# FSSRepo/ggml-cuda-experiments

Hardware: AMD Instinct MI355X
Metric: attn TFLOPS & HBM GB/s per GPU; head_dim=128 seq=4096 Q8_0 KV (higher is better)
Workload: dtype f16; 1 GPU; decode_q8_0_h32_hkv32_d128_n4096_q1; heads=32, kv_heads=32, head_dim=128, kv_len=4096, n_q=1, kv_type=q8_0, kv_layout=head, kv_rotation=16, parallelism=single_gpu

## Files before the change

ggml-cuda-experiments_amd/csrc/fattn_api.hip:

```cpp
#include <hip/hip_runtime.h>

#include <algorithm>
#include <atomic>
#include <cmath>
#include <cstdio>
#include <cstdlib>
#include <cstring>
#include <type_traits>

#include "fattn_plan.h"

using namespace fattn;

namespace {

constexpr int kCUsDefault = 256;

int device_cus() {
    static std::atomic<int> cache[kMaxDevices];
    int dev = 0;
    if (hipGetDevice(&dev) != hipSuccess || dev < 0 || dev >= kMaxDevices) {
        (void)hipGetLastError();
        return kCUsDefault;
    }
// ... 136 lines not shown
            std::snprintf(kern, sizeof kern, "%s<%s,D%d,%s>%s%s", pl.kernel == Kernel::Bdp ? "fattn_bdp_kernel" : "fattn_bd_kernel",
                          tn(pl.kt), pl.D, hm, xcd, merge);
            break;
        case Kernel::Mq:
            if (pl.a.merge_launch)
                std::snprintf(merge, sizeof merge, " + fattn_mq_merge_kernel%s", pl.a.part_f16 ? "(f16 partials)" : "");
            std::snprintf(kern, sizeof kern, "fattn_mq_kernel<%s,D%d,%dwaves,%s>%s", tn(pl.kt), pl.D, pl.nw, hm, merge);
            break;
        case Kernel::Split:
        case Kernel::SplitLd: {
            const bool ld = pl.kernel == Kernel::SplitLd;
            merged_by("fattn_merge_kernel");
            std::snprintf(kern, sizeof kern, "%s<%s,%s,D%d,gran%d,%s,%dwaves%s>%s%s", ld ? "fattn_split_ld_kernel" : "fattn_split_kernel",
                          tn(pl.kt), tn(pl.vt), pl.D, pl.gran, hm, pl.nwv, ld ? "+4loaders" : "", xcd, merge);
            break;
        }
    }
    char planes[48] = "";
    if (pl.a.m_ne2 > 1 || pl.a.m_ne3 > 1) std::snprintf(planes, sizeof planes, " mask planes (%d,%d)", pl.a.m_ne2, pl.a.m_ne3);
    char xf[64] = "";
    int xn = 0;
    if (pl.a.xf.live & 1) xn = std::snprintf(xf, sizeof xf, " softcap %g", (double)p->logit_softcap);
    if (pl.a.xf.live & 2) std::snprintf(xf + xn, sizeof xf - xn, " alibi %g", (double)p->max_bias);
    const int n = std::snprintf(out, cap, "%s grid(%u,%u,%u) lds %d chunk %d steps/slots %d ws %zu%s%s", kern, pl.grid.x,
                                pl.grid.y, pl.grid.z, pl.lds, pl.a.chunk_len, pl.a.nbuf, pl.ws_bytes, planes, xf);
    return n < 0 || (size_t)n >= cap ? FATTN_ERR_INVALID_ARG : FATTN_OK;
}

}

namespace {

int launch_ext(const fattn_params* p, const float* sinks, void* stream, void* ev_begin, void* ev_end) {
    Plan pl;
    const int rc = plan_now(p, pl);
    if (rc != FATTN_OK) return rc;
    if ((uintptr_t)sinks % 4) return FATTN_ERR_ALIGNMENT;
    pl.a.sinks = sinks;
    if (pl.ws_bytes) {
        if (!p->workspace || p->workspace_bytes < pl.ws_bytes || (uintptr_t)p->workspace % 16) return FATTN_ERR_WORKSPACE;
        uint8_t* w = (uint8_t*)p->workspace;
        pl.a.ws_cnt = (uint32_t*)w;
        uint32_t e = g_epoch.fetch_add(1, std::memory_order_relaxed) + 1;
        if (e == 0) e = g_epoch.fetch_add(1, std::memory_order_relaxed) + 1;
        pl.a.arrival_stamp = kArrivalTag | (uint64_t)e << kArrivalEpochShift;
        pl.a.ws_ml = (float*)(w + pl.cnt_bytes);
        pl.a.ws_o = (float*)(w + pl.cnt_bytes + pl.ml_bytes);
        if (pl.pf_flags) pl.a.pf_flags = w;
        if (pl.pf_stage) {
            pl.a.k = w + pl.stage_off;
            pl.a.v = w + pl.stage_off + pl.stage_bytes;
        }
    }
    hipStream_t st = (hipStream_t)stream;
    Events ev;
    ev.begin = (hipEvent_t)ev_begin;
    ev.end = (hipEvent_t)ev_end;
    if (pl.kernel == Kernel::Mla) return launch_mla(pl, st, ev);
    switch (pl.D) {
        case 64: return launch_types<64>(pl, st, ev);
        case 80: return launch_types<80>(pl, st, ev);
        case 96: return launch_types<96>(pl, st, ev);
        case 128: return launch_types<128>(pl, st, ev);
        default: return launch_types<256>(pl, st, ev);
    }
}

}

extern "C" {

int fattn_ext(const fattn_params* p, void* stream) { return launch_ext(p, nullptr, stream, nullptr, nullptr); }

int fattn_ext_events(const fattn_params* p, void* stream, void* ev_begin, void* ev_end) {
    return launch_ext(p, nullptr, stream, ev_begin, ev_end);
}

int fattn_ext_sinks(const fattn_params* p, const float* sinks, void* stream) {
    return launch_ext(p, sinks, stream, nullptr, nullptr);
}

int fattn_ext_f16_launch(const void* q, const void* k, const void* v, const void* mask, float* dst, float scale,
                         int ne00, int ne01, int ne02, int ne03, int ne10, int ne11, int ne12, int ne13, int ne31,
                         int nb31, int nb01, int nb02, int nb03, int nb11, int nb12, int nb13, int ne0, int ne1,
                         int ne2, int ne3, int k_type, int v_type, void* workspace, size_t workspace_bytes,
                         void* stream) {
    (void)ne0; (void)ne1; (void)ne2; (void)ne3;
    if (k_type != v_type) return FATTN_ERR_INVALID_ARG;
    fattn_params p;
    std::memset(&p, 0, sizeof(p));
    p.q = {q, FATTN_TYPE_F32, 0, {ne00, ne01, ne02, ne03}, {4, nb01, nb02, nb03}};
    const int64_t kb0 = k_type == FATTN_TYPE_F16 ? 2 : (int64_t)fattn_row_size(k_type, 32);
    const int64_t vb0 = v_type == FATTN_TYPE_F16 ? 2 : (int64_t)fattn_row_size(v_type, 32);
    p.k = {k, k_type, 0, {ne10, ne11, ne12, ne13}, {kb0, nb11, nb12, nb13}};
    p.v = {v, v_type, 0, {ne10, ne11, ne12, ne13}, {vb0, nb11, nb12, nb13}};
    if (mask)
        p.mask = {mask, FATTN_TYPE_F16, 0, {nb31 / 2, ne31, 1, 1}, {2, nb31, (int64_t)nb31 * ne31, (int64_t)nb31 * ne31}};
    p.dst = dst;
    p.scale = scale;
    p.workspace = workspace;
    p.workspace_bytes = workspace_bytes;
    return fattn_ext(&p, stream);
}

static void fill_row_params(fattn_params& p, const float* query, const void* key, const void* value, const void* mask,
                            float* qkv, int head_dim, int kv_size, int num_heads, float scale, int head_stride,
// ... 132 lines not shown
```

ggml-cuda-experiments_amd/csrc/fattn_plan.h:

```cpp
#pragma once

#include <algorithm>
#include <climits>
#include <cmath>
#include <cstring>
#include <initializer_list>
#include <type_traits>

#include "fattn_launch.h"

namespace fattn {

struct OptionRow {
    int id, def, lo, hi;
    uint64_t set;
    bool flag;
    bool legal(int v) const {
        if (flag) return true;
        if (set) return v >= 0 && v < 64 && (set >> v & 1);
        return v == 0 || (v >= lo && v <= hi);
    }
    int stored(int v) const { return flag ? v != 0 : v; }
};
constexpr OptionRow opt_range(int id, int lo, int hi, int def = 0) { return {id, def, lo, hi, 0, false}; }
// ... 598 lines not shown
    if (nch > 1) {
        const size_t parts = (size_t)S * Y * nch * kMlaRows;
        pl.cnt_bytes = 0;
        pl.ml_bytes = (parts * 2 * sizeof(float) + 255) / 256 * 256;
        pl.ws_bytes = pl.ml_bytes + parts * kMlaDV * 4;
    }
    return FATTN_OK;
}

inline int make_plan(const fattn_params* p, const Options& o, int cus, Plan& pl) {
    Views w;
    const int rc = check_views(p, w);
    if (rc != FATTN_OK) return rc;
    pl = Plan();
    pl.cus = cus;
    pl.merge_plain = o[FATTN_OPT_MERGE_PLAIN] == 2;
    pl.kt = p->k.type;
    pl.vt = w.v_trans ? VT_F16T : p->v.type;
    pl.D = (int)w.D;
    pl.gran = w.g16 ? 16 : 4;
    SplitArgs& a = pl.a;
    fill_args(p, w, a);
    if (w.mla) {
        pl.kernel = Kernel::Mla;
        pl.DV = kMlaDV;
        pl.mla_v_off = (int)w.mla_v_off;
        pack_tiles(a, kMlaRows, (int)std::min<int64_t>(a.rk2, kMlaRows), w.NQ);
        if (pl.kt != FATTN_TYPE_F16) {
            pl.mla_solo = std::min<int64_t>(a.QPT, w.NQ) * a.R <= kRows;
            pl.mla_raw16 = pl.mla_solo && p->k.nb[1] == (int64_t)row_size(pl.kt, kMlaDK) && (uintptr_t)p->k.data % 16 == 0 &&
                           (w.Hkv == 1 || p->k.nb[2] % 16 == 0) && (w.Skv == 1 || p->k.nb[3] % 16 == 0);
        }
        const int64_t Ym = (int64_t)w.Hkv * a.n_hsub * a.n_qt;
        if (Ym > 65535 || w.S > 65535) return FATTN_ERR_INVALID_ARG;
        return size_mla(pl, p->kv_chunk, Ym, w.S, w.N);
    }
    choose_kernel(p, w, o, pl);
    const int64_t Y = (int64_t)w.Hkv * a.n_hsub * a.n_qt;
    if (Y > 65535 || w.S > 65535) return FATTN_ERR_INVALID_ARG;
    switch (pl.kernel) {
        case Kernel::Pf: return size_pf(pl, o, p, w, Y);
        case Kernel::Bd:
        case Kernel::Bdp: return size_bd(pl, o, p->kv_chunk, Y, w.S, w.N);
        case Kernel::Mq: return size_mq(pl, o, p->kv_chunk, Y, w.S, w.N);
        default: break;
    }
    if (w.m_ne2 > 1) {
        a.m_hp = 1;
        if (w.m_span_h + w.m_span + 64 > kSpanMax) return FATTN_ERR_BAD_STRIDE;
    }
    return size_split(pl, o, p->kv_chunk, Y, w.S, w.N, w.NQ);
}

}
```

ggml-cuda-experiments_amd/csrc/fattn_split.h:

```cpp
#pragma once

#include "fattn_common.h"

namespace fattn {

constexpr int kSplitWaves = 4;
constexpr int kStep = 32;
constexpr int kRows = 16;
constexpr int VT_F16T = 100;
constexpr int kCntStride = 64;
constexpr float kRescaleLog2 = 3.0f;
constexpr float kRescaleNat = kRescaleLog2 * 0.6931471805599453f;
#ifdef FATTN_DMA_NO_NT
constexpr bool kDecodeNT = false;
#else
constexpr bool kDecodeNT = true;
#endif

struct SplitArgs {
    const uint8_t* q;
    const uint8_t* k;
    const uint8_t* v;
    const uint8_t* mask;
    float* dst;
    uint32_t* ws_cnt;
    float* ws_o;
    float* ws_ml;
    int64_t q_nb1, q_nb2, q_nb3;
    int64_t k_nb1, k_nb2, k_nb3;
    int64_t v_nb0, v_nb1, v_nb2, v_nb3;
    int64_t m_nb1;
    int64_t m_nb2, m_nb3;
    int m_ne2, m_ne3;
    float m_ne2_inv;
    uint32_t m_span_h;
    int m_hp;
    int m_hg;
    uint32_t k_span, v_span, m_span, q_span;
    int NQ, H, S;
    int N;
    int rk2, rk3;
    int R;
    int QPT;
    int n_hsub, n_qt;
    float R_inv;
    int chunk_len;
    int n_chunks;
    int ncp;
    float scale_log2;
    float scale;
    int has_mask;
    int nbuf;
    int wave_bytes;
    int pf_stagger;
    const uint8_t* pf_flags;
    int split_prio;
    int wave_merge;
    uint64_t arrival_stamp;
    int merge_launch;
    int step_skip;
    int xcd_group;
    int part_f16;
    ScoreXf xf;
    const float* sinks;
};

__host__ __device__ constexpr int swz_mask(int cpr) { return (cpr & -cpr) - 1; }

template <int D>
constexpr int epi_ept() { return (D / 16) % 4 == 0 ? D / 16 : 8; }

template <int KT, int VT, int D>
struct SplitCfg {
    static constexpr int KTT = KT;
    static constexpr int VTT = (VT == VT_F16T) ? FATTN_TYPE_F16 : VT;
    static constexpr int rowK = row_bytes<KT, D>();
    static constexpr int rowV = row_bytes<VTT, D>();
    static constexpr int kBytes = kStep * rowK;
    static constexpr int vBytes = kStep * rowV;
    static constexpr int mBytes = kRows * kStep * 2;
    static constexpr int stepBytes = (kBytes + vBytes + mBytes + 15) / 16 * 16;
    static constexpr int vscBytes = 0;
    static constexpr int kMergeStride = D + 4;
    static constexpr int mergeBytes = kRows * kMergeStride * 4 + kRows * 2 * 4;
    static constexpr int wave_bytes(int nbuf) {
        const int w = (nbuf * stepBytes + vscBytes + 15) / 16 * 16;
        return w > mergeBytes ? w : mergeBytes;
    }
    static constexpr int lds_bytes(int nbuf) { return kSplitWaves * wave_bytes(nbuf); }
};

template <int N>
__device__ __forceinline__ void wait_vmcnt_c() {
    static_assert(N >= 0, "");
    constexpr int n = N > 63 ? 63 : N;
    asm volatile("s_waitcnt vmcnt(%0)" ::"n"(n) : "memory");
}

template <int NI>
__device__ __forceinline__ void wait_steps(int outstanding) {
    switch (__builtin_amdgcn_readfirstlane(outstanding)) {
        case 0: wait_vmcnt_c<0>(); break;
        case 1: wait_vmcnt_c<NI>(); break;
        case 2: wait_vmcnt_c<2 * NI>(); break;
        default: wait_vmcnt_c<3 * NI>(); break;
    }
}

template <int NI, int EXTRA>
__device__ __forceinline__ void wait_steps_plus(int outstanding) {
    switch (__builtin_amdgcn_readfirstlane(outstanding)) {
        case 0: wait_vmcnt_c<EXTRA>(); break;
        case 1: wait_vmcnt_c<NI + EXTRA>(); break;
        case 2: wait_vmcnt_c<2 * NI + EXTRA>(); break;
        default: wait_vmcnt_c<3 * NI + EXTRA>(); break;
    }
}

template <int KT, int VT, int D, int GRAN>
struct StepPlan {
    using C = SplitCfg<KT, VT, D>;
    static constexpr int PK = C::kBytes / GRAN;
    static constexpr int PV = C::vBytes / GRAN;
    static constexpr int NIK = (PK + kWave - 1) / kWave;
    static constexpr int NIV = (PV + kWave - 1) / kWave;
    static constexpr int NIKV = NIK + NIV;
    static constexpr int MG = GRAN == 16 ? 16 : 4;
    static constexpr int MPR = kStep * 2 / MG;
    static constexpr int PM = kRows * MPR;
    static constexpr int NIM = PM / kWave;
    static_assert(PM % kWave == 0, "");
};

typedef __attribute__((address_space(3))) void lds_void;
typedef int i32x4 __attribute__((ext_vector_type(4)));

__device__ __forceinline__ i32x4 make_srd(const void* base, uint32_t bytes) {
    const uint64_t p = (uint64_t)base;
    i32x4 r;
    r.x = __builtin_amdgcn_readfirstlane((int)(uint32_t)p);
    r.y = __builtin_amdgcn_readfirstlane((int)(uint32_t)(p >> 32));
    r.z = __builtin_amdgcn_readfirstlane((int)bytes);
    r.w = 0x00020000;
    return r;
}

__device__ __forceinline__ uint32_t lds_addr(const void* p) { return (uint32_t)(uintptr_t)(const lds_void*)p; }

__device__ __forceinline__ __amdgpu_buffer_rsrc_t make_rsrc(const void* base, uint32_t bytes) {
    const uint64_t p = (uint64_t)base;
    const uint32_t lo = __builtin_amdgcn_readfirstlane((uint32_t)p);
    const uint32_t hi = __builtin_amdgcn_readfirstlane((uint32_t)(p >> 32));
    const uint32_t n = __builtin_amdgcn_readfirstlane(bytes);
    return __builtin_amdgcn_make_buffer_rsrc((void*)(((uint64_t)hi << 32) | lo), 0, (int)n, 0x00020000);
}
constexpr int kAuxSc1 = 16;

__device__ __forceinline__ u32x4 ld_sc1_buf(__amdgpu_buffer_rsrc_t r, uint32_t off) {
    return __builtin_bit_cast(u32x4, __builtin_amdgcn_raw_buffer_load_b128(r, off, 0, kAuxSc1));
}
__device__ __forceinline__ uint32_t ld_sc1_buf_b32(__amdgpu_buffer_rsrc_t r, uint32_t off) {
    return __builtin_amdgcn_raw_buffer_load_b32(r, off, 0, kAuxSc1);
}

enum : int { kTagQ = 1, kTagMaskWords = 2 };
template <int TAG>
__device__ __forceinline__ u32x4 ld_buf_untracked(const i32x4& srd, uint32_t off) {
    u32x4 v;
// ... 63 lines not shown
    const uint32_t gen = (uint32_t)(old >> 16) & 0xFFu;
    if ((int)(old & 0xFFFF) == n - 1) {
        __hip_atomic_store(w, (old & ~0xFFFFFFull) | (uint64_t)((gen + 1) & 0xFFu) << 16, __ATOMIC_RELAXED,
                           __HIP_MEMORY_SCOPE_AGENT);
        return 1;
    }
    for (uint32_t spins = 0; spins < (1u << 20); spins++) {
        const uint32_t lo = ld_sc1_u32((const uint32_t*)w);
        if (((lo >> 16) & 0xFFu) != gen || (int)(lo & 0xFFFF) >= n) return 1;
        __builtin_amdgcn_s_sleep(2);
    }
    return 0;
}

__device__ __forceinline__ int div_R(const SplitArgs& a, int m);

__device__ __forceinline__ const uint8_t* mask_seq_base(const SplitArgs& a, int iq3) {
    return a.m_ne3 == 1 ? a.mask : a.mask + (int64_t)(iq3 % a.m_ne3) * a.m_nb3;
}

__device__ __forceinline__ uint32_t mask_head_off(const SplitArgs& a, int iq2) {
    if (a.m_ne2 == 1) return 0u;
    int r = iq2 - (int)(((float)iq2 + 0.5f) * a.m_ne2_inv) * a.m_ne2;
    r = r < 0 ? r + a.m_ne2 : r >= a.m_ne2 ? r - a.m_ne2 : r;
    return (uint32_t)r * (uint32_t)a.m_nb2;
}

template <bool HM>
__device__ __forceinline__ void split_mask_src(const SplitArgs& a, StepSrc& rs, int iq3, int ik2, int hs) {
    rs.m = make_srd(mask_seq_base(a, iq3), HM ? a.m_span_h : 0);
    rs.mh0 = ik2 * a.rk2 + hs * a.R;
    rs.mhn = min(a.R, a.rk2 - hs * a.R);
    rs.mrows = a.m_hp ? kRows : a.QPT;
}

__device__ __forceinline__ uint32_t mask_row_off(const SplitArgs& a, const StepSrc& rs, int mrow0, int r) {
    if (!a.m_hp) return (uint32_t)(mrow0 + r) * (uint32_t)a.m_nb1;
    const int rq = div_R(a, r), hh = r - rq * a.R;
    const bool ok = rq < a.QPT && mrow0 + rq < a.NQ && hh < rs.mhn;
    return ok ? (uint32_t)(mrow0 + rq) * (uint32_t)a.m_nb1 + mask_head_off(a, rs.mh0 + hh) : a.m_span_h;
}

template <int KT, int VT, int D, int GRAN>
__device__ __forceinline__ void mask_lane_offsets(const SplitArgs& a, const StepSrc& rs, int mrow0, int lane,
                                                  uint32_t (&ml)[StepPlan<KT, VT, D, GRAN>::NIM]) {
    using P = StepPlan<KT, VT, D, GRAN>;
#pragma unroll
    for (int i = 0; i < P::NIM; i++) {
        const int q = i * kWave + lane;
        ml[i] = mask_row_off(a, rs, mrow0, q / P::MPR) + (q % P::MPR) * P::MG;
    }
}

template <int KT, int VT, int D, int GRAN, bool HM>
__device__ __forceinline__ void issue_step(const SplitArgs& a, const StepSrc& rs, int n0,
                                           const uint32_t (&ml)[StepPlan<KT, VT, D, GRAN>::NIM], uint8_t* buf,
                                           int lane, bool kv_live = true) {
#ifdef FATTN_DIAG_NOMEM
    return;
#endif
    using C = SplitCfg<KT, VT, D>;
    using P = StepPlan<KT, VT, D, GRAN>;
    const uint32_t kn1 = (uint32_t)a.k_nb1, vn1 = (uint32_t)a.v_nb1;
    i32x4 ksrd = rs.k, vsrd = rs.v;
    ksrd.z = __builtin_amdgcn_readfirstlane(kv_live ? rs.k.z : 0);
    vsrd.z = __builtin_amdgcn_readfirstlane(kv_live ? rs.v.z : 0);
#pragma unroll
    for (int i = 0; i < P::NIK; i++) {
        const int p = i * kWave + lane;
        const int byte = p * GRAN;
        uint32_t off;
        if constexpr (KT == FATTN_TYPE_F16) {
            constexpr int SW = swz_mask(C::rowK / 16);
            const int row = byte / C::rowK;
            const int chunk = ((byte % C::rowK) / 16) ^ (row & SW);
            off = (uint32_t)(n0 + row) * kn1 + chunk * 16 + (byte & 15);
        } else if constexpr (GRAN == 16) {
            off = (uint32_t)n0 * C::rowK + byte;
        } else {
            const int row = byte / C::rowK;
            off = (uint32_t)(n0 + row) * kn1 + (byte % C::rowK);
        }
        if (P::PK % kWave == 0 || p < P::PK) dma<GRAN, kDecodeNT>(ksrd, lds_addr(buf + i * kWave * GRAN), off);
    }
    if constexpr (HM) {
        uint8_t* mbuf = buf + C::kBytes + C::vBytes;
#pragma unroll
        for (int i = 0; i < P::NIM; i++) {
            const int mr = (i * kWave + lane) / P::MPR;
            const uint32_t moff = ml[i] + (uint32_t)n0 * 2;
            if (GRAN != 16 || mr < rs.mrows) dma<P::MG>(rs.m, lds_addr(mbuf + i * kWave * P::MG), moff);
        }
    }
    uint8_t* vbuf = buf + C::kBytes;
#pragma unroll
    for (int i = 0; i < P::NIV; i++) {
        const int p = i * kWave + lane;
        const int byte = p * GRAN;
        uint32_t off;
        if constexpr (VT == VT_F16T) {
            const int d = byte / (kStep * 2);
            off = (uint32_t)d * (uint32_t)a.v_nb0 + (uint32_t)n0 * 2 + (byte % (kStep * 2));
        } else if constexpr (VT == FATTN_TYPE_F16) {
            constexpr int SW = swz_mask(C::rowV / 16);
            const int row = byte / C::rowV;
            const int chunk = ((byte % C::rowV) / 16) ^ (((row & 7) << 1) & SW);
            off = (uint32_t)(n0 + row) * vn1 + chunk * 16 + (byte & 15);
        } else if constexpr (GRAN == 16) {
            off = (uint32_t)n0 * C::rowV + byte;
        } else {
            const int row = byte / C::rowV;
            off = (uint32_t)(n0 + row) * vn1 + (byte % C::rowV);
        }
        if (P::PV % kWave == 0 || p < P::PV) dma<GRAN, kDecodeNT>(vsrd, lds_addr(vbuf + i * kWave * GRAN), off);
    }
}

template <int VT>
constexpr int v_code_centre() { return VT == FATTN_TYPE_Q4_1 ? 8 : VT == FATTN_TYPE_Q5_1 ? 16 : 0; }
template <int VT>
constexpr float v_code_off() {
    return VT == FATTN_TYPE_Q8_0 ? 1152.0f : VT == FATTN_TYPE_Q4_0 ? 1032.0f : VT == FATTN_TYPE_Q5_0 ? 1040.0f
           : 1024.0f + (float)v_code_centre<VT>();
}
template <int VT, int D>
constexpr int corr_len() { return (D + QK - 1) / QK * (has_min(VT) ? 2 : 1); }

template <int VT, int EPI>
constexpr bool col_packed() { return EPI != 0 && (VT == FATTN_TYPE_Q8_0 || VT == FATTN_TYPE_Q4_0); }
template <int VT, int D, bool CP>
constexpr int corr_regs() { return CP ? 1 : corr_len<VT, D>(); }

template <int T, int D>
struct RowScales {
    uint32_t w[D / QK];
};
template <int T, int D>
__host__ __device__ constexpr bool scale_hi(int b) {
    return row_bytes<T, D>() % 4 == 0 && ((TypeInfo<T>::block_bytes * b) & 2) != 0;
}
template <int T, int D>
__device__ __forceinline__ RowScales<T, D> row_scales(const uint8_t* row) {
    constexpr int BB = TypeInfo<T>::block_bytes;
    RowScales<T, D> s;
#pragma unroll
    for (int b = 0; b < D / QK; b++) {
        if constexpr (row_bytes<T, D>() % 4 != 0) s.w[b] = *(const uint16_t*)(row + BB * b);
        else s.w[b] = *(const uint32_t*)(row + ((BB * b) & ~3));
    }
    return s;
}
template <int T, int D>
__device__ __forceinline__ uint32_t scale_bits(const RowScales<T, D>& s, int b) {
    return scale_hi<T, D>(b) ? (s.w[b] >> 16) : (s.w[b] & 0xffffu);
}
template <int T, int D>
__device__ __forceinline__ uint32_t scale_bcast(const RowScales<T, D>& s, int b) {
    return perm_b32(s.w[b], s.w[b], scale_hi<T, D>(b) ? 0x03020302u : 0x01000100u);
}
template <int T, int D>
__device__ __forceinline__ f16x2 scale_pair(const RowScales<T, D>& s0, const RowScales<T, D>& s1, int b) {
    constexpr int BB = TypeInfo<T>::block_bytes;
    return as_h2(((BB * b) & 2) ? perm_b32(s1.w[b], s0.w[b], 0x07060302u) : perm_b32(s1.w[b], s0.w[b], 0x05040100u));
}

__device__ __forceinline__ u32x2 read8_any(const uint8_t* smem, uint32_t off) {
    const uint32_t base = off & ~3u, sh = off & 3u;
    const uint32_t w0 = *(const uint32_t*)(smem + base);
// ... 132 lines not shown
    const int heads = min(a.R, a.rk2 - hs * a.R);
    return rows_q * heads;
}

#ifdef FATTN_STAMPS
static __device__ unsigned long long* g_stamps;
#define FATTN_STAMP(k)                                                                          \
    do {                                                                                        \
        if (lane == 0 && g_stamps) {                                                            \
            const unsigned long long t_ = __builtin_amdgcn_s_memrealtime();                     \
            const int64_t blk_ = ((int64_t)blockIdx.z * gridDim.y + blockIdx.y) * gridDim.x + blockIdx.x; \
            g_stamps[(blk_ * 16 + wave) * 16 + (k)] = t_;                                \
        }                                                                                       \
    } while (0)
#define FATTN_STAMP_MAX(k, v)                                                                   \
    do {                                                                                        \
        if (g_stamps) {                                                                         \
            const int64_t blk_ = ((int64_t)blockIdx.z * gridDim.y + blockIdx.y) * gridDim.x + blockIdx.x; \
            atomicMax(&g_stamps[blk_ * 16 * 16 + (k)], (unsigned long long)(v));      \
        }                                                                                       \
    } while (0)
__device__ __forceinline__ unsigned long long* split_stamp_slots() {
    __shared__ unsigned long long s[16 * 16];
    return s;
}
#define FATTN_SSTAMP(k)                                                                          \
    do {                                                                                         \
        if (lane == 0) split_stamp_slots()[wave * 16 + (k)] = __builtin_amdgcn_s_memrealtime();  \
    } while (0)
#define FATTN_SSTAMP_INIT()                                                                      \
    do {                                                                                         \
        if (lane < 16) split_stamp_slots()[wave * 16 + lane] = 0ull;                             \
    } while (0)
#define FATTN_SSTAMP_FLUSH()                                                                     \
    do {                                                                                         \
        if (lane < 16 && g_stamps) {                                                             \
            const int64_t blk_ = ((int64_t)blockIdx.z * gridDim.y + blockIdx.y) * gridDim.x + blockIdx.x; \
            g_stamps[(blk_ * 16 + wave) * 16 + lane] = split_stamp_slots()[wave * 16 + lane];    \
        }                                                                                        \
    } while (0)
#else
#define FATTN_STAMP(k) do { } while (0)
#define FATTN_STAMP_MAX(k, v) do { } while (0)
#define FATTN_SSTAMP(k) do { } while (0)
#define FATTN_SSTAMP_INIT() do { } while (0)
#define FATTN_SSTAMP_FLUSH() do { } while (0)
#endif


__device__ __forceinline__ void tile_coords(const SplitArgs& a, int& chunk, int& y, int& iq3) {
    chunk = blockIdx.x;
    y = blockIdx.y;
    iq3 = blockIdx.z;
    if (a.xcd_group) {
        const uint32_t gx = gridDim.x, gy = gridDim.y;
        const uint32_t G = gx * gy * gridDim.z;
        const uint32_t L = blockIdx.x + gx * (blockIdx.y + gy * blockIdx.z);
        const uint32_t L2 = (L % 8) * (G / 8) + L / 8;
        chunk = (int)(L2 % gx);
        y = (int)((L2 / gx) % gy);
        iq3 = (int)(L2 / (gx * gy));
    }
}


template <int D, int CB = 2>
__device__ __forceinline__ void combine_tile(const SplitArgs& a, int64_t tile, int qt, int hs, int ik2, int iq3,
                                             int rv, int row_base, uint8_t* smem);

constexpr int kWaveMergeParts = 64;
constexpr int kWaveMergeBatch = 32;
template <int D, bool VQ8, int NW = kSplitWaves, bool CP = false>
__device__ __forceinline__ void wave_merge_epilogue(const SplitArgs& a, const f32x4 (&o)[D / 16], float m_run,
                                                    float l_tot, int chunk, int wave, int lane, int qt, int hs,
                                                    int ik2, int iq3, int y) {
    static_assert(D == 128, "lane i <-> dims 2i, 2i+1");
    constexpr int NB = D / QK;
    constexpr int NC = D / 16;
    constexpr float kNegInf = -__builtin_inff();
    const int g = lane >> 4, m = lane & 15;
    const int NP = a.n_chunks * NW;
    const int64_t tile = (int64_t)iq3 * gridDim.y + y;
    const int part = chunk * NW + wave;
    float* po = a.ws_o + (tile * NP + part) * D;
    auto bits = [](float x) { return __builtin_bit_cast(uint32_t, x); };
    if constexpr (CP) {
#pragma unroll
        for (int b = 0; b < NB; b++) {
            if (m != b) continue;
            if constexpr (VQ8) {
                const f32x4 e = o[2 * b], od = o[2 * b + 1];
                st_sc1(po + 32 * b + 8 * g, u32x4{bits(e.x), bits(od.x), bits(e.y), bits(od.y)});
                st_sc1(po + 32 * b + 8 * g + 4, u32x4{bits(e.z), bits(od.z), bits(e.w), bits(od.w)});
            } else {
#pragma unroll
                for (int c = 2 * b; c < 2 * b + 2; c++)
                    st_sc1(po + 16 * c + 4 * g, u32x4{bits(o[c].x), bits(o[c].y), bits(o[c].z), bits(o[c].w)});
            }
        }
        if (lane == 0) st_sc1_x2(a.ws_ml + 2 * (tile * NP + part), u32x2{bits(m_run), bits(l_tot)});
    } else if (m == 0) {
        if constexpr (VQ8) {
#pragma unroll
            for (int b = 0; b < NB; b++) {
                const f32x4 e = o[2 * b], od = o[2 * b + 1];
                st_sc1(po + 32 * b + 8 * g, u32x4{bits(e.x), bits(od.x), bits(e.y), bits(od.y)});
                st_sc1(po + 32 * b + 8 * g + 4, u32x4{bits(e.z), bits(od.z), bits(e.w), bits(od.w)});
            }
        } else {
#pragma unroll
            for (int c = 0; c < NC; c++)
                st_sc1(po + 16 * c + 4 * g, u32x4{bits(o[c].x), bits(o[c].y), bits(o[c].z), bits(o[c].w)});
        }
        if (g == 0) st_sc1_x2(a.ws_ml + 2 * (tile * NP + part), u32x2{bits(m_run), bits(l_tot)});
// ... 747 lines not shown
                if constexpr (has_qh(VTT)) {
                    const int HO = BB * b + qh_off(VTT);
#pragma unroll
                    for (int r = 0; r < 8; r++) {
                        const uint8_t* hp = vb + ((r < 4 ? rA : rB - 4) + r) * C::rowV + HO;
                        uint32_t qh;
                        if (HO % 4 == 0) qh = *(const uint32_t*)hp;
                        else qh = (uint32_t)*(const uint16_t*)hp | ((uint32_t)*(const uint16_t*)(hp + 2) << 16);
                        hb[r] = (qh >> i16) & 0x00010001u;
                    }
                }
                u32x4 al, ah;
#pragma unroll
                for (int pr = 0; pr < 4; pr++) {
                    const uint32_t x = w[2 * pr] | (w[2 * pr + 1] << 16);
                    al[pr] = (x & 0x000F000Fu) | 0x64006400u;
                    ah[pr] = ((x >> 4) & 0x000F000Fu) | 0x64006400u;
                    if constexpr (has_qh(VTT)) {
                        al[pr] |= perm_b32(hb[2 * pr + 1], hb[2 * pr], 0x0c040c00u) << 4;
                        ah[pr] |= perm_b32(hb[2 * pr + 1], hb[2 * pr], 0x0c060c02u) << 4;
                    }
                }
                o[2 * b] = mfma16(__builtin_bit_cast(f16x8, al), pbd, o[2 * b]);
                o[2 * b + 1] = mfma16(__builtin_bit_cast(f16x8, ah), pbd, o[2 * b + 1]);
            }
        }
    }

}

template <int KT, int D, int GRAN>
constexpr int split_waves_per_simd() {
    return (KT == FATTN_TYPE_F16 || GRAN == 4 || D == 256 || is_kv_ext(KT)) ? 2 : 4;
}

template <int KT, int VT, int D, int GRAN, bool HM, int NWV, int EPI, bool XF = false>
__global__ __launch_bounds__(NWV * kWave, (KT == FATTN_TYPE_F16 || GRAN == 4 || D == 256 || is_kv_ext(KT)) ? 2 : 4) void fattn_split_kernel(
    const SplitArgs a) {
    using C = SplitCfg<KT, VT, D>;
    using P = StepPlan<KT, VT, D, GRAN>;
    constexpr int NI = P::NIKV + (HM ? P::NIM : 0);
    extern __shared__ __attribute__((aligned(16))) uint8_t smem[];
    constexpr int NB = (D + QK - 1) / QK;
    constexpr int NC = D / 16;
    constexpr float kNegInf = -__builtin_inff();

    const int lane = threadIdx.x & 63;
    const int wave = __builtin_amdgcn_readfirstlane(threadIdx.x >> 6);
    const int g = lane >> 4;
    const int i16 = lane & 15;
    FATTN_SSTAMP_INIT();
    FATTN_SSTAMP(0);

    int chunk, y, iq3;
    tile_coords(a, chunk, y, iq3);
    int qt = 0, hs = 0, ik2 = y, ik3 = iq3;
    if (a.n_qt != 1 || a.n_hsub != 1) {
        qt = y % a.n_qt;
        hs = (y / a.n_qt) % a.n_hsub;
        ik2 = y / (a.n_qt * a.n_hsub);
    }
    if (a.rk3 != 1) ik3 = iq3 / a.rk3;

    constexpr bool CP = col_packed<C::VTT, EPI>();
    const int m = (CP && i16 < D / QK) ? 0 : i16;
    const int mq = div_R(a, m);
    const int mh = hs * a.R + (m - mq * a.R);
    const int iq1 = qt * a.QPT + mq;
    const int iq2 = ik2 * a.rk2 + mh;
    const bool row_ok = (m < a.QPT * a.R) && (iq1 < a.NQ) && (mh < a.rk2);
    const int mrow = a.m_hp ? m : (mq < a.QPT ? mq : 0);
    const float slope = XF ? xf_slope(a.xf, iq2) : 1.0f;

    const int wl = a.chunk_len / NWV;
    const int c_hi = min(a.N, (chunk + 1) * a.chunk_len);
    const int w_lo = chunk * a.chunk_len + wave * wl;
    const int w_hi = min(c_hi, w_lo + wl);
    const int nsteps = w_hi > w_lo ? (w_hi - w_lo + kStep - 1) / kStep : 0;
    const int nbuf = a.nbuf;

    StepSrc rs;
    rs.k = make_srd(a.k + (int64_t)ik2 * a.k_nb2 + (int64_t)ik3 * a.k_nb3, a.k_span);
    rs.v = make_srd(a.v + (int64_t)ik2 * a.v_nb2 + (int64_t)ik3 * a.v_nb3, a.v_span);
    split_mask_src<HM>(a, rs, iq3, ik2, hs);
    uint8_t* wbuf = smem + wave * a.wave_bytes;
    const int mrow0 = qt * a.QPT;
    uint32_t ml[P::NIM];
    mask_lane_offsets<KT, VT, D, GRAN>(a, rs, mrow0, lane, ml);

    if (a.split_prio != 1) {
        switch (__builtin_amdgcn_readfirstlane(NWV == 4 ? wave : wave >> 2)) {
            case 0: __builtin_amdgcn_s_setprio(3); break;
            case 1: __builtin_amdgcn_s_setprio(2); break;
            case 2: __builtin_amdgcn_s_setprio(1); break;
            default: break;
        }
    }

    u32x4 qraw[NB][2];
    {
        const i32x4 qs = make_srd(a.q + (int64_t)iq3 * a.q_nb3, a.q_span);
        const uint32_t qoff = row_ok ? (uint32_t)iq1 * (uint32_t)a.q_nb1 + (uint32_t)iq2 * (uint32_t)a.q_nb2 + 32 * g
                                     : a.q_span;
#pragma unroll
        for (int b = 0; b < NB; b++) {
            const uint32_t qb = (D % QK == 0 || 32 * b + 8 * g < D) ? qoff + 128 * b : a.q_span;
            qraw[b][0] = ld_buf_untracked<kTagQ>(qs, qb);
            qraw[b][1] = ld_buf_untracked<kTagQ>(qs, qb + 16);
        }
    }
    const int pro = min(nbuf, nsteps);
    const int n_rows = !HM ? 0 : a.m_hp ? tile_rows(a, qt, hs) : min(a.QPT, a.NQ - mrow0);
    const bool pre = HM && a.step_skip && nsteps >= 4 && n_rows * nsteps <= kWave;
    u32x4 mraw[4] = {};
    if (pre) {
        const int r = lane / nsteps, st = lane - r * nsteps;
        const uint32_t moff = r < n_rows ? mask_row_off(a, rs, mrow0, r) + (uint32_t)(w_lo + st * kStep) * 2
                                         : a.m_span_h;
#pragma unroll
        for (int j = 0; j < 4; j++) mraw[j] = ld_buf_untracked<kTagMaskWords>(rs.m, moff + 16 * j);
    }
    for (int s = 0; s < pro; s++) {
        issue_step<KT, VT, D, GRAN, HM>(a, rs, w_lo + s * kStep, ml, wbuf + s * C::stepBytes, lane);
    }
    if (a.n_chunks > 1 && a.merge_launch != 1 && lane == 0 && (EPI == 1 || wave == 0))
        arrival_begin(a, (int64_t)iq3 * gridDim.y + y);

    FATTN_SSTAMP(1);
    if (a.split_prio == 2) __builtin_amdgcn_s_setprio(0);
    wait_steps<NI>(pro);
#pragma unroll
    for (int b = 0; b < NB; b++) {
        reg_fence<kTagQ>(qraw[b][0]);
        reg_fence<kTagQ>(qraw[b][1]);
    }
#pragma unroll
    for (int j = 0; j < 4; j++) reg_fence<kTagMaskWords>(mraw[j]);
    f16x8 qop[NB];
#pragma unroll
    for (int b = 0; b < NB; b++) {
        const f32x4 x0 = __builtin_bit_cast(f32x4, qraw[b][0]), x1 = __builtin_bit_cast(f32x4, qraw[b][1]);
        f16x8 h;
        h.s0 = (f16)x0.x; h.s1 = (f16)x0.y; h.s2 = (f16)x0.z; h.s3 = (f16)x0.w;
        h.s4 = (f16)x1.x; h.s5 = (f16)x1.y; h.s6 = (f16)x1.z; h.s7 = (f16)x1.w;
        qop[b] = h;
    }
    uint64_t live = ~0ull;
    if (pre) {
        constexpr uint32_t kNegInf2 = 0xFC00FC00u;
        bool lv = false;
#pragma unroll
        for (int j = 0; j < 4; j++) {
            lv |= (mraw[j].x != kNegInf2) | (mraw[j].y != kNegInf2) | (mraw[j].z != kNegInf2) | (mraw[j].w != kNegInf2);
        }
        const uint64_t bl = __builtin_amdgcn_ballot_w64(lv && lane < n_rows * nsteps);
        live = 0;
        for (int r = 0; r < n_rows; r++) live |= bl >> (r * nsteps);
    }

    float m_run = kNegInf;
    float l_run = 0.0f;
    f32x4 o[NC];
#pragma unroll
    for (int c = 0; c < NC; c++) o[c] = f32x4{0, 0, 0, 0};
    float corr[corr_regs<VT, D, CP>()];
#pragma unroll
    for (int b = 0; b < corr_regs<VT, D, CP>(); b++) corr[b] = 0.0f;

    int cur = 0;
    for (int s = 0; s < nsteps; s++) {
        const int ahead = min(nbuf - 1, nsteps - 1 - s);
        wait_steps_plus<NI, P::NIV>(ahead);
        if (s < 8) FATTN_SSTAMP(2 + s);
#ifdef FATTN_DIAG_NOCOMPUTE
        wait_steps<NI>(ahead);
        if (s + nbuf < nsteps) {
            issue_step<KT, VT, D, GRAN, HM>(a, rs, w_lo + (s + nbuf) * kStep, ml, wbuf + cur * C::stepBytes, lane);
        }
        cur = (cur + 1 == nbuf) ? 0 : cur + 1;
        continue;
#endif
        const int n0 = w_lo + s * kStep;
        int s_opaque = s;
// ... 305 lines not shown
```

Measured before the change: 3374 GB/s.

## Issue first K step early using a host-packed hot argument block

Adds a 128-byte SplitHot block of kernel arguments filled on the host, holding the K/V pointers, strides, chunk geometry, flags and a precomputed magic-division tile map. The split kernel reads these to compute its wave range and issue the first step's K DMA before the Q load, mask setup and the V/mask DMA. The wait count is reduced by the K instructions to match the new issue order. The XCD remap swaps runtime integer division for multiply-shift division. The aim is to start HBM traffic sooner at kernel entry and to trim scalar prologue work. The cost is some duplicated argument data and more complex vmcnt accounting that must match the split issue order.

```diff
diff --git a/ggml-cuda-experiments_amd/csrc/fattn_api.hip b/ggml-cuda-experiments_amd/csrc/fattn_api.hip
--- a/ggml-cuda-experiments_amd/csrc/fattn_api.hip
+++ b/ggml-cuda-experiments_amd/csrc/fattn_api.hip
@@ -212,6 +212,7 @@
             pl.a.v = w + pl.stage_off + pl.stage_bytes;
         }
     }
+    fill_hot(pl);
     hipStream_t st = (hipStream_t)stream;
     Events ev;
     ev.begin = (hipEvent_t)ev_begin;
diff --git a/ggml-cuda-experiments_amd/csrc/fattn_plan.h b/ggml-cuda-experiments_amd/csrc/fattn_plan.h
--- a/ggml-cuda-experiments_amd/csrc/fattn_plan.h
+++ b/ggml-cuda-experiments_amd/csrc/fattn_plan.h
@@ -674,4 +674,22 @@
     return size_split(pl, o, p->kv_chunk, Y, w.S, w.N, w.NQ);
 }
 
-}
+inline void fill_hot(Plan& pl) {
+    SplitArgs& a = pl.a;
+    SplitHot& h = a.hot;
+    h = SplitHot();
+    h.k = a.k, h.v = a.v;
+    h.k_nb2 = a.k_nb2, h.k_nb3 = a.k_nb3, h.v_nb2 = a.v_nb2, h.v_nb3 = a.v_nb3;
+    h.k_span = a.k_span, h.v_span = a.v_span;
+    h.k_nb1 = (uint32_t)a.k_nb1, h.v_nb1 = (uint32_t)a.v_nb1;
+    h.chunk_len = a.chunk_len, h.N = a.N, h.nbuf = a.nbuf, h.wave_bytes = a.wave_bytes;
+    h.wl = pl.nwv > 0 ? a.chunk_len / pl.nwv : 0;
+    const uint64_t G = (uint64_t)pl.grid.x * pl.grid.y * pl.grid.z;
+    const bool xcd = a.xcd_group && G % 8 == 0 && G < (1ull << 32);
+    h.tm = make_tile_map(pl.grid.x, pl.grid.y, pl.grid.z);
+    h.flags = (a.n_qt != 1 || a.n_hsub != 1 ? kHotTileDiv : 0u) | (a.rk3 != 1 ? kHotRk3 : 0u) | (xcd ? kHotXcd : 0u) |
+              (a.m_ne3 != 1 ? kHotMaskSeq : 0u) | (a.m_hp ? kHotMaskHp : 0u) | ((uint32_t)(a.split_prio & 3) << kHotPrioShift) |
+              (a.n_chunks > 1 && a.merge_launch != 1 ? kHotArrive : 0u);
+}
+
+}
diff --git a/ggml-cuda-experiments_amd/csrc/fattn_split.h b/ggml-cuda-experiments_amd/csrc/fattn_split.h
--- a/ggml-cuda-experiments_amd/csrc/fattn_split.h
+++ b/ggml-cuda-experiments_amd/csrc/fattn_split.h
@@ -1,6 +1,7 @@
 #pragma once
 
 #include "fattn_common.h"
+#include "fattn_tilemap.h"
 
 namespace fattn {
 
@@ -16,6 +17,29 @@
 #else
 constexpr bool kDecodeNT = true;
 #endif
+
+enum : uint32_t {
+    kHotTileDiv = 1u << 0,
+    kHotRk3 = 1u << 1,
+    kHotXcd = 1u << 2,
+    kHotMaskSeq = 1u << 3,
+    kHotMaskHp = 1u << 4,
+    kHotPrioShift = 5,
+    kHotArrive = 1u << 7,
+};
+struct alignas(64) SplitHot {
+    const uint8_t* k;
+    const uint8_t* v;
+    int64_t k_nb2, k_nb3, v_nb2, v_nb3;
+    uint32_t k_span, v_span;
+    uint32_t flags;
+    int wl;
+    TileMap tm;
+    int chunk_len, N, nbuf, wave_bytes;
+    uint32_t k_nb1, v_nb1;
+    uint32_t pad_[2];
+};
+static_assert(sizeof(SplitHot) == 128, "two 64-B lines");
 
 struct SplitArgs {
     const uint8_t* q;
@@ -63,6 +87,7 @@
     int part_f16;
     ScoreXf xf;
     const float* sinks;
+    SplitHot hot;
 };
 
 __host__ __device__ constexpr int swz_mask(int cpr) { return (cpr & -cpr) - 1; }
@@ -114,6 +139,17 @@
         case 1: wait_vmcnt_c<NI + EXTRA>(); break;
         case 2: wait_vmcnt_c<2 * NI + EXTRA>(); break;
         default: wait_vmcnt_c<3 * NI + EXTRA>(); break;
+    }
+}
+
+template <int NI, int LESS>
+__device__ __forceinline__ void wait_steps_less(int steps) {
+    static_assert(LESS >= 0 && LESS <= NI, "");
+    switch (__builtin_amdgcn_readfirstlane(steps)) {
+        case 0: wait_vmcnt_c<0>(); break;
+        case 1: wait_vmcnt_c<NI - LESS>(); break;
+        case 2: wait_vmcnt_c<2 * NI - LESS>(); break;
+        default: wait_vmcnt_c<3 * NI - LESS>(); break;
     }
 }
 
@@ -283,19 +319,17 @@
     }
 }
 
-template <int KT, int VT, int D, int GRAN, bool HM>
-__device__ __forceinline__ void issue_step(const SplitArgs& a, const StepSrc& rs, int n0,
-                                           const uint32_t (&ml)[StepPlan<KT, VT, D, GRAN>::NIM], uint8_t* buf,
-                                           int lane, bool kv_live = true) {
+template <int KT, int VT, int D, int GRAN>
+__device__ __forceinline__ void issue_step_k(const SplitArgs& a, const i32x4& k, int n0, uint8_t* buf, int lane,
+                                             bool kv_live = true) {
 #ifdef FATTN_DIAG_NOMEM
     return;
 #endif
     using C = SplitCfg<KT, VT, D>;
     using P = StepPlan<KT, VT, D, GRAN>;
-    const uint32_t kn1 = (uint32_t)a.k_nb1, vn1 = (uint32_t)a.v_nb1;
-    i32x4 ksrd = rs.k, vsrd = rs.v;
-    ksrd.z = __builtin_amdgcn_readfirstlane(kv_live ? rs.k.z : 0);
-    vsrd.z = __builtin_amdgcn_readfirstlane(kv_live ? rs.v.z : 0);
+    const uint32_t kn1 = a.hot.k_nb1;
+    i32x4 ksrd = k;
+    ksrd.z = __builtin_amdgcn_readfirstlane(kv_live ? k.z : 0);
 #pragma unroll
     for (int i = 0; i < P::NIK; i++) {
         const int p = i * kWave + lane;
@@ -314,6 +348,20 @@
         }
         if (P::PK % kWave == 0 || p < P::PK) dma<GRAN, kDecodeNT>(ksrd, lds_addr(buf + i * kWave * GRAN), off);
     }
+}
+
+template <int KT, int VT, int D, int GRAN, bool HM>
+__device__ __forceinline__ void issue_step_mv(const SplitArgs& a, const StepSrc& rs, int n0,
+                                              const uint32_t (&ml)[StepPlan<KT, VT, D, GRAN>::NIM], uint8_t* buf,
+                                              int lane, bool kv_live = true) {
+#ifdef FATTN_DIAG_NOMEM
+    return;
+#endif
+    using C = SplitCfg<KT, VT, D>;
+    using P = StepPlan<KT, VT, D, GRAN>;
+    const uint32_t vn1 = a.hot.v_nb1;
+    i32x4 vsrd = rs.v;
+    vsrd.z = __builtin_amdgcn_readfirstlane(kv_live ? rs.v.z : 0);
     if constexpr (HM) {
         uint8_t* mbuf = buf + C::kBytes + C::vBytes;
 #pragma unroll
@@ -345,6 +393,14 @@
         }
         if (P::PV % kWave == 0 || p < P::PV) dma<GRAN, kDecodeNT>(vsrd, lds_addr(vbuf + i * kWave * GRAN), off);
     }
+}
+
+template <int KT, int VT, int D, int GRAN, bool HM>
+__device__ __forceinline__ void issue_step(const SplitArgs& a, const StepSrc& rs, int n0,
+                                           const uint32_t (&ml)[StepPlan<KT, VT, D, GRAN>::NIM], uint8_t* buf,
+                                           int lane, bool kv_live = true) {
+    issue_step_k<KT, VT, D, GRAN>(a, rs.k, n0, buf, lane, kv_live);
+    issue_step_mv<KT, VT, D, GRAN, HM>(a, rs, n0, ml, buf, lane, kv_live);
 }
 
 template <int VT>
@@ -583,14 +639,12 @@
     chunk = blockIdx.x;
     y = blockIdx.y;
     iq3 = blockIdx.z;
-    if (a.xcd_group) {
-        const uint32_t gx = gridDim.x, gy = gridDim.y;
-        const uint32_t G = gx * gy * gridDim.z;
-        const uint32_t L = blockIdx.x + gx * (blockIdx.y + gy * blockIdx.z);
-        const uint32_t L2 = (L % 8) * (G / 8) + L / 8;
-        chunk = (int)(L2 % gx);
-        y = (int)((L2 / gx) % gy);
-        iq3 = (int)(L2 / (gx * gy));
+    if (a.hot.flags & kHotXcd) {
+        uint32_t c2, y2, z2;
+        tile_remap(a.hot.tm, blockIdx.x, blockIdx.y, blockIdx.z, c2, y2, z2);
+        chunk = (int)c2;
+        y = (int)y2;
+        iq3 = (int)z2;
     }
 }
 
@@ -1444,15 +1498,44 @@
     FATTN_SSTAMP_INIT();
     FATTN_SSTAMP(0);
 
+    const SplitHot& hot = a.hot;
+    const uint32_t hflags = hot.flags;
+    asm volatile("" ::"s"(hot.chunk_len), "s"(hot.N), "s"(hot.nbuf), "s"(hot.wave_bytes), "s"(hot.wl));
+    asm volatile("" ::"s"(a.q), "s"(a.q_nb1), "s"(a.m_nb1), "s"(a.q_span), "s"(a.scale));
     int chunk, y, iq3;
     tile_coords(a, chunk, y, iq3);
     int qt = 0, hs = 0, ik2 = y, ik3 = iq3;
-    if (a.n_qt != 1 || a.n_hsub != 1) {
+    if (hflags & kHotTileDiv) {
         qt = y % a.n_qt;
         hs = (y / a.n_qt) % a.n_hsub;
         ik2 = y / (a.n_qt * a.n_hsub);
     }
-    if (a.rk3 != 1) ik3 = iq3 / a.rk3;
+    if (hflags & kHotRk3) ik3 = iq3 / a.rk3;
+
+    const int wl = hot.wl;
+    const int c_hi = min(hot.N, (chunk + 1) * hot.chunk_len);
+    const int w_lo = chunk * hot.chunk_len + wave * wl;
+    const int w_hi = min(c_hi, w_lo + wl);
+    const int nsteps = w_hi > w_lo ? (w_hi - w_lo + kStep - 1) / kStep : 0;
+    const int nbuf = hot.nbuf;
+    const int pro = min(nbuf, nsteps);
+
+    StepSrc rs;
+    rs.k = make_srd(hot.k + (int64_t)ik2 * hot.k_nb2 + (int64_t)ik3 * hot.k_nb3, hot.k_span);
+    rs.v = make_srd(hot.v + (int64_t)ik2 * hot.v_nb2 + (int64_t)ik3 * hot.v_nb3, hot.v_span);
+    uint8_t* wbuf = smem + wave * hot.wave_bytes;
+
+    const uint32_t prio = (hflags >> kHotPrioShift) & 3u;
+    if (prio != 1) {
+        switch (__builtin_amdgcn_readfirstlane(NWV == 4 ? wave : wave >> 2)) {
+            case 0: __builtin_amdgcn_s_setprio(3); break;
+            case 1: __builtin_amdgcn_s_setprio(2); break;
+            case 2: __builtin_amdgcn_s_setprio(1); break;
+            default: break;
+        }
+    }
+    if (pro > 0) issue_step_k<KT, VT, D, GRAN>(a, rs.k, w_lo, wbuf, lane);
+    __builtin_amdgcn_sched_barrier(0);
 
     constexpr bool CP = col_packed<C::VTT, EPI>();
     const int m = (CP && i16 < D / QK) ? 0 : i16;
@@ -1461,33 +1544,6 @@
     const int iq1 = qt * a.QPT + mq;
     const int iq2 = ik2 * a.rk2 + mh;
     const bool row_ok = (m < a.QPT * a.R) && (iq1 < a.NQ) && (mh < a.rk2);
-    const int mrow = a.m_hp ? m : (mq < a.QPT ? mq : 0);
-    const float slope = XF ? xf_slope(a.xf, iq2) : 1.0f;
-
-    const int wl = a.chunk_len / NWV;
-    const int c_hi = min(a.N, (chunk + 1) * a.chunk_len);
-    const int w_lo = chunk * a.chunk_len + wave * wl;
-    const int w_hi = min(c_hi, w_lo + wl);
-    const int nsteps = w_hi > w_lo ? (w_hi - w_lo + kStep - 1) / kStep : 0;
-    const int nbuf = a.nbuf;
-
-    StepSrc rs;
-    rs.k = make_srd(a.k + (int64_t)ik2 * a.k_nb2 + (int64_t)ik3 * a.k_nb3, a.k_span);
-    rs.v = make_srd(a.v + (int64_t)ik2 * a.v_nb2 + (int64_t)ik3 * a.v_nb3, a.v_span);
-    split_mask_src<HM>(a, rs, iq3, ik2, hs);
-    uint8_t* wbuf = smem + wave * a.wave_bytes;
-    const int mrow0 = qt * a.QPT;
-    uint32_t ml[P::NIM];
-    mask_lane_offsets<KT, VT, D, GRAN>(a, rs, mrow0, lane, ml);
-
-    if (a.split_prio != 1) {
-        switch (__builtin_amdgcn_readfirstlane(NWV == 4 ? wave : wave >> 2)) {
-            case 0: __builtin_amdgcn_s_setprio(3); break;
-            case 1: __builtin_amdgcn_s_setprio(2); break;
-            case 2: __builtin_amdgcn_s_setprio(1); break;
-            default: break;
-        }
-    }
 
     u32x4 qraw[NB][2];
     {
@@ -1501,7 +1557,8 @@
             qraw[b][1] = ld_buf_untracked<kTagQ>(qs, qb + 16);
         }
     }
-    const int pro = min(nbuf, nsteps);
+    split_mask_src<HM>(a, rs, iq3, ik2, hs);
+    const int mrow0 = qt * a.QPT;
     const int n_rows = !HM ? 0 : a.m_hp ? tile_rows(a, qt, hs) : min(a.QPT, a.NQ - mrow0);
     const bool pre = HM && a.step_skip && nsteps >= 4 && n_rows * nsteps <= kWave;
     u32x4 mraw[4] = {};
@@ -1512,15 +1569,20 @@
 #pragma unroll
         for (int j = 0; j < 4; j++) mraw[j] = ld_buf_untracked<kTagMaskWords>(rs.m, moff + 16 * j);
     }
-    for (int s = 0; s < pro; s++) {
+    const int mrow = a.m_hp ? m : (mq < a.QPT ? mq : 0);
+    const float slope = XF ? xf_slope(a.xf, iq2) : 1.0f;
+    uint32_t ml[P::NIM];
+    mask_lane_offsets<KT, VT, D, GRAN>(a, rs, mrow0, lane, ml);
+    if (pro > 0) issue_step_mv<KT, VT, D, GRAN, HM>(a, rs, w_lo, ml, wbuf, lane);
+    for (int s = 1; s < pro; s++) {
         issue_step<KT, VT, D, GRAN, HM>(a, rs, w_lo + s * kStep, ml, wbuf + s * C::stepBytes, lane);
     }
-    if (a.n_chunks > 1 && a.merge_launch != 1 && lane == 0 && (EPI == 1 || wave == 0))
+    if ((hflags & kHotArrive) && lane == 0 && (EPI == 1 || wave == 0))
         arrival_begin(a, (int64_t)iq3 * gridDim.y + y);
 
     FATTN_SSTAMP(1);
-    if (a.split_prio == 2) __builtin_amdgcn_s_setprio(0);
-    wait_steps<NI>(pro);
+    if (prio == 2) __builtin_amdgcn_s_setprio(0);
+    wait_steps_less<NI, P::NIK>(pro);
 #pragma unroll
     for (int b = 0; b < NB; b++) {
         reg_fence<kTagQ>(qraw[b][0]);
diff --git a/ggml-cuda-experiments_amd/csrc/fattn_tilemap.h b/ggml-cuda-experiments_amd/csrc/fattn_tilemap.h
--- /dev/null
+++ b/ggml-cuda-experiments_amd/csrc/fattn_tilemap.h
@@ -0,0 +1,54 @@
+#pragma once
+
+#include <stdint.h>
+
+#ifdef __HIPCC__
+#define FATTN_TM_FN __host__ __device__ __forceinline__
+#else
+#define FATTN_TM_FN inline
+#endif
+
+namespace fattn {
+
+struct TileMap {
+    uint32_t gx, gy;
+    uint32_t g8;
+    uint32_t mx, sx;
+    uint32_t my, sy;
+    uint32_t pad_;
+};
+
+FATTN_TM_FN uint32_t tm_div(uint32_t n, uint32_t mul, uint32_t sh) {
+    const uint32_t t = (uint32_t)(((uint64_t)mul * n) >> 32);
+    return (t + ((n - t) >> (sh & 0xFF))) >> (sh >> 8);
+}
+
+FATTN_TM_FN void tm_make_div(uint32_t d, uint32_t& mul, uint32_t& sh) {
+    uint32_t l = 0;
+    while (l < 32 && ((uint64_t)1 << l) < d) l++;
+    mul = (uint32_t)(((((uint64_t)1 << l) - d) << 32) / d + 1);
+    const uint32_t sh1 = l < 1 ? l : 1;
+    sh = sh1 | (l - sh1) << 8;
+}
+
+FATTN_TM_FN TileMap make_tile_map(uint32_t gx, uint32_t gy, uint32_t gz) {
+    TileMap tm = {};
+    tm.gx = gx;
+    tm.gy = gy;
+    tm.g8 = (uint32_t)((uint64_t)gx * gy * gz / 8);
+    tm_make_div(gx, tm.mx, tm.sx);
+    tm_make_div(gy, tm.my, tm.sy);
+    return tm;
+}
+
+FATTN_TM_FN void tile_remap(const TileMap& tm, uint32_t bx, uint32_t by, uint32_t bz, uint32_t& chunk, uint32_t& y,
+                            uint32_t& z) {
+    const uint32_t L = bx + tm.gx * (by + tm.gy * bz);
+    const uint32_t L2 = (L & 7) * tm.g8 + (L >> 3);
+    const uint32_t t = tm_div(L2, tm.mx, tm.sx);
+    chunk = L2 - t * tm.gx;
+    z = tm_div(t, tm.my, tm.sy);
+    y = t - z * tm.gy;
+}
+
+}
```

New measurement: 3420 GB/s (median of 6 runs). 1.01x the previous value.
